# TensorSpeech/TensorFlowASR

Hardware: AMD Instinct MI355X
Metric: audio-hours/sec (train step) Conformer-M RNN-T (higher is better)
Workload: dtype bf16; 1 GPU; Conformer-M transducer full train step (fwd+RNN-T loss+bwd+Adam), LibriSpeech-shaped 16 kHz utterances, 32/GPU, padding=batch, SpecAugment on, dropout 0.1; global_batch=32, parallelism=dp1, params=32461288

## Files before the change

include/tfasr_hip.h:

```cpp
#ifndef TFASR_HIP_H_
#define TFASR_HIP_H_

#include <stddef.h>
#include <stdint.h>

#ifdef __cplusplus
extern "C" {
#endif

#define TFASR_ABI_VERSION 44

typedef enum {
  TFASR_STATUS_SUCCESS = 0,
  TFASR_STATUS_INVALID_VALUE = 1,
  TFASR_STATUS_EXECUTION_FAILED = 2,
  TFASR_STATUS_UNSUPPORTED = 3
} tfasr_status_t;

typedef enum { TFASR_F32 = 0, TFASR_BF16 = 1 } tfasr_dtype_t;

const char* tfasr_status_string(int status);
int tfasr_abi_version(void);
size_t tfasr_launch_count(void);

// ... 37 lines not shown
  void* prez;
  int M, N, K;
  int lda, ldb, ldd;
  int trans_a, trans_b;
  int nb1, nb2;
  long sA1, sA2, sB1, sB2, sD1, sD2;
  float alpha, beta;
  int act;
  int dact;
  int dtype;
  int out_f32;
  int accumulate;
  int split_k;
  float drop_p;
  long drop_seed;
  float* ws;
  long ws_elems;
  float* colsum;
  float* lse_part; int lse_parts; const int32_t* row_label; float* pick;
  const long* seg_a_off; const long* seg_b_off; int seg_k;
  const float* rgrad_coef;
  const void* bns_x; const float* bns_fin; float* bns_out; int bns_copies;
  int bns_c;
} tfasr_gemm_args;

int tfasr_gemm(const tfasr_gemm_args* args, void* stream);
int tfasr_gemm_group(const tfasr_gemm_args* args, int n, void* stream);

int tfasr_layernorm_fwd(const void* x, const float* gamma, const float* beta, void* y, float* mean, float* rstd,
                        long rows, int C, float eps, int dtype, void* stream);
int tfasr_ffn_fused_fwd(const void* x, const float* gamma, const float* beta, const void* W1, const float* b1, const void* W2,
                        const float* b2, void* y, void* ln, float* mean, float* rstd, void* z, void* h, long rows, int d, int F,
                        float ln_eps, float res_factor, float drop_p, long drop_seed1, long drop_seed2, int dtype, void* stream);
int tfasr_ffn_fused_fwd2(const void* x, const float* gamma, const float* beta, const void* W1, const float* b1, const void* W2,
                         const float* b2, void* y, void* ln, float* mean, float* rstd, void* z, int z_factor, void* h, long rows, int d, int F,
                         float ln_eps, float res_factor, float drop_p, long drop_seed1, long drop_seed2, int dtype, void* stream);
int tfasr_ln_dense_fwd(const void* x, const float* gamma, const float* beta, const void* W, const float* b, void* out, void* ln, float* mean,
                       float* rstd, long rows, int d, int N, float ln_eps, int dtype, void* stream);
int tfasr_layernorm_bwd(const void* dy, const void* x, const float* gamma, const float* mean, const float* rstd,
                        const void* add, void* dx, float* dgamma, float* dbeta, long rows, int C, int dtype,
                        void* stream);
int tfasr_layernorm_bwd_drop(const void* dy, const void* x, const float* gamma, const float* mean, const float* rstd,
                             const void* add, void* dx, float* dgamma, float* dbeta, void* dx_dropped, float drop_p,
                             long drop_seed, long rows, int C, int dtype, void* stream);
int tfasr_layernorm_bwd_part_blocks(long rows, int C, int dtype);
int tfasr_layernorm_bwd_part(const void* dy, const void* x, const float* gamma, const float* mean, const float* rstd, const void* add,
// ... 175 lines not shown
int tfasr_conv1_bwd_weight(const void* x, const void* dy, float* dw, float* db, int B, int T0, int F0, int C,
                           int dtype, void* stream);
int tfasr_conv1_fwd_s2d(const void* x, const float* w, const float* bias, void* y, int B, int T0, int F0, int C, int dtype,
                        void* stream);
int tfasr_conv1_bwd_weight_s2d(const void* x, const void* dy, float* dw, float* db, int B, int T0, int F0, int C, int dtype,
                               void* stream);
int tfasr_conv1_stats(const void* x, const float* w, const float* bias, float* stats, int B, int T0, int F0, int C, int dtype,
                      void* stream);
int tfasr_conv1_bn_apply_s2d(const void* x, const float* w, const float* bias, const float* fin, void* y, int B, int T0, int F0, int C,
                             int dtype, void* stream);
int tfasr_conv1_bn_bwd_stats_s2d(const void* x, const float* w, const float* bias, const float* fin, const void* dy, float* bstats, int B,
                                 int T0, int F0, int C, int dtype, void* stream);
int tfasr_conv1_bn_bwd_apply_s2d(const void* x, const float* w, const float* bias, const float* fin, const float* bstats, float count,
                                 const void* dy, float* dw, float* db, int B, int T0, int F0, int C, int dtype, void* stream);
#define TFASR_CONV1_GRAM_DOUBLES 768
int tfasr_conv1_gram(const void* x, double* gram, int B, int T0, int F0, int dtype, void* stream);
int tfasr_conv1_stats_from_gram(const double* gram, const float* w, const float* bias, float* stats, int C, void* stream);
int tfasr_conv1_bn_bwd_onepass_s2d(const void* x, const float* w, const float* bias, const float* fin, const void* dy, float* bstats,
                                   float* pbuf, int B, int T0, int F0, int C, int dtype, void* stream);
int tfasr_conv1_bn_bwd_finalize(const double* gram, const float* w, const float* bias, const float* fin, const float* bstats, float count,
                                const float* pbuf, float* dw, float* db, int C, void* stream);
int tfasr_halo_zero(void* x, int B, int T2, int F2, int W, int dtype, void* stream);
int tfasr_s2d_edge_zero(void* x, int B, int T1, int F1, int C, int dtype, void* stream);
int tfasr_im2col_3x3s2(const void* x, void* col, int B, int T1, int F1, int C, int dtype, void* stream);
int tfasr_col2im_3x3s2(const void* dcol, void* dx, int B, int T1, int F1, int C, int dtype, void* stream);

int tfasr_logmel(const float* signal, int B, int N, float preemph, const float* window, int frame_len, int frame_step,
                 int nfft, const float* melw, const int32_t* band, int F, float eps, void* out, int T0, int dtype,
                 void* stream);

int tfasr_rows_subsample_fwd(const void* x, void* y, int B, int T, int C, int stride, int dtype, void* stream);
int tfasr_rows_subsample_bwd(const void* dy, void* dx, int B, int T, int C, int stride, int dtype, void* stream);
int tfasr_se_pool(const void* x, const int32_t* lengths, float* pool, int B, int T, int C, int dtype, void* stream);
int tfasr_se_scale_fwd(const void* x, const float* scale, void* y, int B, int T, int C, int dtype, void* stream);
int tfasr_se_scale_bwd_reduce(const void* x, const void* dy, float* dscale, int B, int T, int C, int dtype, void* stream);
int tfasr_se_bwd_apply(const void* dy, const float* scale, const float* dpool, const int32_t* lengths, void* dx, int B, int T,
                       int C, int dtype, void* stream);
int tfasr_add_act_fwd(const void* a, const void* b, void* y, long n, int act, int dtype, void* stream);
int tfasr_add_act_bwd(const void* a, const void* b, const void* dy, void* d, long n, int act, int dtype, void* stream);

int tfasr_ctc_beam_search_host(const float* logits, const int32_t* logit_len, int B, int T, int V, int beam_width,
                               int blank_index, int32_t* tokens, int32_t* tokens_len, float* log_prob);

int tfasr_ctc_beam_search_workspace_size(int B, int T, int V, int beam_width, size_t* bytes);
int tfasr_ctc_beam_search(const void* logits, const int32_t* logit_len, int B, int T, int V, int beam_width, int top_paths,
                          int blank_index, int dtype, int32_t* tokens, int32_t* tokens_len, float* log_prob, void* workspace,
// ... 216 lines not shown
```

tensorflowasr_amd/_lib.py:

```python
import ctypes
import os
from ctypes import POINTER, Structure, c_char_p, c_float, c_int, c_int32, c_long, c_size_t, c_void_p

HERE = os.path.dirname(os.path.abspath(__file__))
LIB_PATH = os.environ.get("TFASR_LIB") or os.path.join(HERE, "lib", "libtfasr_hip.so")

TFASR_F32, TFASR_BF16 = 0, 1
ACT_NONE, ACT_SWISH, ACT_TANH, ACT_SIGMOID, ACT_TANH_OUT, ACT_FACTOR = 0, 1, 2, 3, 4, 5


class TfasrError(RuntimeError):
    pass


class GemmArgs(Structure):
    _fields_ = [
        ("A", c_void_p), ("B", c_void_p), ("D", c_void_p),
        ("bias", c_void_p), ("res", c_void_p), ("dact_z", c_void_p), ("prez", c_void_p),
        ("M", c_int), ("N", c_int), ("K", c_int),
        ("lda", c_int), ("ldb", c_int), ("ldd", c_int),
        ("trans_a", c_int), ("trans_b", c_int),
        ("nb1", c_int), ("nb2", c_int),
        ("sA1", c_long), ("sA2", c_long), ("sB1", c_long), ("sB2", c_long), ("sD1", c_long), ("sD2", c_long),
        ("alpha", c_float), ("beta", c_float),
        ("act", c_int), ("dact", c_int), ("dtype", c_int), ("out_f32", c_int), ("accumulate", c_int), ("split_k", c_int),
        ("drop_p", c_float), ("drop_seed", c_long),
        ("ws", c_void_p), ("ws_elems", c_long), ("colsum", c_void_p),
        ("lse_part", c_void_p), ("lse_parts", c_int), ("row_label", c_void_p), ("pick", c_void_p),
        ("seg_a_off", c_void_p), ("seg_b_off", c_void_p), ("seg_k", c_int),
        ("rgrad_coef", c_void_p),
        ("bns_x", c_void_p), ("bns_fin", c_void_p), ("bns_out", c_void_p), ("bns_copies", c_int), ("bns_c", c_int),
    ]


BLOCK_PARAM_NAMES = [
    "ff1/ln/g", "ff1/ln/b", "ff1/d1/w", "ff1/d1/b", "ff1/d2/w", "ff1/d2/b",
    "ff2/ln/g", "ff2/ln/b", "ff2/d1/w", "ff2/d1/b", "ff2/d2/w", "ff2/d2/b",
    "mhsa/ln/g", "mhsa/ln/b", "mhsa/qkv/w", "mhsa/qkv/b", "mhsa/pos/w", "mhsa/pos/b", "mhsa/o/w", "mhsa/o/b", "/enc/u", "/enc/v",
    "conv/ln/g", "conv/ln/b", "conv/pw1/w", "conv/pw1/b", "conv/dw/w", "conv/dw/b", "conv/bn/g", "conv/bn/b", "conv/pw2/w", "conv/pw2/b",
    "ln/g", "ln/b",
]
PHASE_A, PHASE_B = 1, 2


class BlockCfg(Structure):
    _fields_ = [
        ("B", c_int), ("T", c_int), ("d", c_int), ("H", c_int), ("dh", c_int), ("dff", c_int), ("ksize", c_int),
        ("dtype", c_int), ("training", c_int), ("save", c_int), ("use_mask", c_int), ("force_unfused", c_int), ("world", c_int),
        ("site0", c_int), ("drop_epoch", c_long),
        ("drop_p", c_float), ("ffm_res", c_float), ("mhsa_res", c_float), ("conv_res", c_float), ("ln_eps", c_float), ("bn_eps", c_float),
        ("bn_momentum", c_float),
        ("chunk_size", c_int), ("history_size", c_int), ("dw_norm_layer", c_int), ("dh_logical", c_int),
    ]

# ... 105 lines not shown
```

tensorflowasr_amd/conformer.py:

```python
import math
import os

import numpy as np
import torch

from . import kernels as K
from .base_model import BaseModel
from .kernels import ACT_NONE, ACT_SWISH, ACT_TANH_OUT
from .params import ParamStore
from .schemas import AlignOutput, PredictInput, PredictOutput, RecognizeOutput, TrainData, TrainInput, TrainOutput


class SingleProcess:

    world = 1
    rank = 0

    def allreduce_stats_(self, t):
        return t

    def set_reduce(self, on):
        pass

    def grads_ready(self, lo, hi):
# ... 11 lines not shown
    return (v + 4) // 8 * 8 if v >= 12 else v


class ConformerTransducer(BaseModel):
    def __init__(self, cfg, device=None, dtype=torch.bfloat16, seed=0, dp=None):
        if not torch.cuda.is_available():
            raise K._lib.TfasrError("ConformerTransducer needs an MI355X (HIP) device; there is no CPU fallback")
        self.cfg = cfg
        self.device = torch.device("cuda", torch.cuda.current_device()) if device is None else torch.device(device)
        self.dtype = dtype
        pad = (dtype == torch.bfloat16 and cfg.head_size < 64 and getattr(cfg, "encoder", "conformer") == "conformer"
               and os.environ.get("TFASR_HEAD_PAD", "1") != "0")
        cpad = (dtype == torch.bfloat16 and cfg.filters % 64 != 0 and getattr(cfg, "encoder", "conformer") == "conformer"
                and getattr(cfg, "sub_norm", "batch") == "batch" and os.environ.get("TFASR_FILTER_PAD", "1") != "0")
        self.ps = ParamStore(cfg, self.device, dtype, seed, head_phys=64 if pad else None, filt_phys=-(-cfg.filters // 64) * 64 if cpad else None)
        self.dp = dp or SingleProcess()
        self.blank = cfg.blank
        self.time_reduction_factor = cfg.time_reduction_factor
        self.step = 0
        self._consts = {}
        self._bn1_sums_in_gemm = True
        self._bn_stats_copies = 8
        self._conv1_gram = True
        self._rng = np.random.default_rng([seed + 1000, int(self.dp.rank)])
        prio = -1
        self.pred_stream = torch.cuda.Stream(device=self.device, priority=prio)
        self.use_pred_stream = os.environ.get("TFASR_NO_PRED_STREAM", "0") != "1"
        self._dp_force_split = os.environ.get("TFASR_DP_FORCE_SPLIT", "0") == "1" and not isinstance(self.dp, SingleProcess)
        self._lstm_persist_auto = os.environ.get("TFASR_LSTM_PERSIST") is None
        self.optimizer = dict(beta1=0.9, beta2=0.98, eps=1e-9, weight_decay=1e-6, schedule=dict(
            dmodel=cfg.dmodel, warmup_steps=10000, scale=2.0, max_lr=0.05 / math.sqrt(cfg.dmodel)))
        self.ga_steps = 1
        self.prefetched_inputs = False
        self._ga_count = 0
        self._drop_epoch = 0
        self.native_blocks = os.environ.get("TFASR_NATIVE_BLOCK", "1") != "0"
        self.wgrad_stream = {"0": False, "1": True}.get(os.environ.get("TFASR_WGRAD_STREAM"), None)
        self._wgrad_keep = []
        self._blk_params, self._blk_sizes = {}, {}
        self._zero_pool = {}
        self.block_hoist = {"0": False, "1": True}.get(os.environ.get("TFASR_BLOCK_HOIST"), None)
        self.dpext_aux = True
        self.joint_wgrad_aux = False
        self._aux_pending = False
        if self.device.type != "cuda":
            self.aux_stream = None
# ... 60 lines not shown
            return None
        return K.matmul(dy, W, trans_b=True, alpha=alpha, dact_z=dact_z, dact=dact, drop_p=drop[0], drop_seed=drop[1])

    def _h2d(self, x, dtype=torch.int32):
        t = x if isinstance(x, torch.Tensor) else torch.as_tensor(np.asarray(x))
        t = t.to(dtype)
        if t.device.type == "cpu":
            if self.device.type == "cuda":
                t = t.pin_memory()
            t = t.to(self.device, non_blocking=True)
        return t

    def frontend(self, signals, signals_length, training=False, masks=None):
        c = self.cfg
        window, melw, band = self._frontend_consts()
        feats = K.logmel(signals, window, melw, band, c.frame_step, c.nfft, c.preemphasis, c.epsilon, self.dtype)
        flen = [-(-int(n) // c.frame_step) for n in signals_length]
        if training:
            if masks is None:
                masks = self.draw_specaugment(flen)
            fm, tm = masks
            if fm is not None or tm is not None:
                K.specaugment(feats, None if fm is None else self._h2d(fm), None if tm is None else self._h2d(tm), 0.0)
        return feats, flen

    def draw_specaugment(self, flen):
        c = self.cfg
        fcfg, tcfg = c.freq_masking, c.time_masking
        B = len(flen)
        rng = self._rng
        nf = fcfg.get("num_masks", 0) if fcfg else 0
        nt = tcfg.get("num_masks", 0) if tcfg else 0
        fm = np.zeros((B, nf, 2), np.int32) if nf > 0 else None
        tm = np.zeros((B, nt, 2), np.int32) if nt > 0 else None
        nb = c.num_feature_bins
        rnd, rint = rng.random, rng.integers
        fprob = fcfg.get("prob", 1.0) if fcfg else 1.0
        fmax = max(1, int(fcfg["mask_factor"])) if nf > 0 else 1
        tprob = tcfg.get("prob", 1.0) if tcfg else 1.0
        tup = np.float32(tcfg.get("p_upperbound", 1.0)) if tcfg else np.float32(1.0)
        for b in range(B):
            ln = int(flen[b])
            for k in range(nf):
                do = 1 if rnd() <= fprob else 0
                f = do * min(int(rint(0, fmax)), nb)
                fm[b, k] = (do * int(rint(0, max(1, nb - f))), f)
            if nt > 0:
# ... 105 lines not shown
                gram = K.conv1_gram(feats, torch.empty(K.CONV1_GRAM_DOUBLES, dtype=torch.float64, device=self.device))
                K.conv1_stats_from_gram(gram, w0, b0, stats)
            else:
                K.conv1_stats(feats, w0, b0, stats)
            count0 = B * T1 * F1 * self.dp.world
            self.dp.allreduce_stats_(stats[:2 * C])
            K.bn_finalize(stats, count0, ps.p(nm + "/g"), ps.p(nm + "/b"), fin0, ps.state[nm + "/mm"], ps.state[nm + "/mv"], 0.99, 1e-3, True)
        else:
            count0 = B * T1 * F1
            K.bn_finalize(None, 1, ps.p(nm + "/g"), ps.p(nm + "/b"), fin0, ps.state[nm + "/mm"], ps.state[nm + "/mv"], 0.99, 1e-3, False)
        a1_full, a1 = self._salloc(rows, 4 * C, slack, tag="a1")
        K.conv1_bn_apply_s2d(feats, w0, b0, fin0, a1)
        K.halo_zero(a1, B, T2, F2, 4 * C)
        K.s2d_edge_zero(a1, B, T1, F1, C)
        bn0 = (fin0, count0, gram)
        W = ps.w2d("enc/sub/conv1/w")
        _, o = self._salloc(rows, C, slack, tag="o")
        if self.dtype == torch.float32:
            flat, base = a1_full, slack * 4 * C
            for i in range(9):
                K.gemm(flat[base + shift[i] * 4 * C + blk[i] * C:], W[i * C:(i + 1) * C], o, rows, C, C, 4 * C, C, C,
                       bias=ps.p("enc/sub/conv1/b") if i == 0 else None, accumulate=i > 0)
        else:
            K.gemm(a1, W, o, rows, C, 9 * C, 4 * C, C, C, bias=ps.p("enc/sub/conv1/b"), seg=fwd_a)
        K.halo_zero(o, B, T2, F2, C)
        _, a2 = self._salloc(rows, C, 0)
        _, bn1 = self._bn_fwd(o, "enc/sub/bn1", training, ACT_SWISH, rows=B * T2 * F2, y=a2)
        K.halo_zero(a2, B, T2, F2, C)
        drop = self._drop(0, training)
        d = c.dmodel
        x0 = torch.empty(B * T2, d, dtype=self.dtype, device=self.device)
        a2flat = a2.view(-1)
        K.gemm(a2flat[((F2 + 1) + 1) * C:], ps.w2d("enc/linear/w"), x0, T2, d, F2 * C, (F2 + 1) * C, d, d, bias=ps.p("enc/linear/b"),
               nb1=B, sA=((T2 + 1) * (F2 + 1) * C, 0), sD=(T2 * d, 0), drop_p=drop[0], drop_seed=drop[1])
        elen = [-(-(-(-n // 2)) // 2) for n in flen]
        if ctx is not None:
            ctx["sub"] = dict(s2d=True, feats=feats, bn0=bn0, a1=a1, a1_full=a1_full, o=o, bn1=bn1, a2=a2,
                              dims=(B, T0, F0, T1, F1, T2, F2), drop=drop)
        return x0, T2, elen

    def _subsampling_bwd_s2d(self, dx0, ctx):
        ps, c = self.ps, self.cfg
        s = ctx["sub"]
        B, T0, F0, T1, F1, T2, F2 = s["dims"]
        C, d = ps.filt_phys, c.dmodel
        rows, slack = B * (T2 + 1) * (F2 + 1), F2 + 2
        shift, blk, _, dgrad = self._seg_tables(F2, C)
# ... 1277 lines not shown
```

tensorflowasr_amd/csrc/conv2d.hip:

```cpp
#include "common.h"
#include <type_traits>
#include <algorithm>

namespace {

inline int flat_grid(long n) { return (int)std::max<long>(1, std::min<long>((n + 255) / 256, 256L * 32)); }

__device__ __forceinline__ long s2d_off(int b, int t, int f, int T2, int F2, int C) {
  return ((((long)b * (T2 + 1) + (t >> 1) + 1) * (F2 + 1) + (f >> 1) + 1) * 4 + ((t & 1) * 2 + (f & 1))) * C;
}

template <typename T>
__global__ __launch_bounds__(256) void conv1_fwd_kernel(const T* __restrict__ x, const float* __restrict__ w,
                                                        const float* __restrict__ bias, T* __restrict__ y, int B, int T0,
                                                        int F0, int T1, int F1, int C, int s2d) {
  const int c8n = C / 8;
  const long n8 = (long)B * T1 * F1 * c8n;
  const long i0 = (long)blockIdx.x * blockDim.x + threadIdx.x;
  const long stride = (long)gridDim.x * blockDim.x;
  const int c = (int)(i0 % c8n) * 8;
  float wr[9][8], br[8];
#pragma unroll
  for (int k = 0; k < 8; ++k) br[k] = bias ? bias[c + k] : 0.f;
#pragma unroll
// ... 516 lines not shown
  for (long i = (long)blockIdx.x * blockDim.x + threadIdx.x; i < n; i += (long)gridDim.x * blockDim.x) {
    const int c8 = (int)(i % w8);
    long r = i / w8;
    const int k = (int)(r % per_b), b = (int)(r / per_b);
    const int tt = k <= F2 ? 0 : k - F2, ff = k <= F2 ? k : 0;
    st8(x + (((long)b * (T2 + 1) + tt) * (F2 + 1) + ff) * W + (long)c8 * 8, z);
  }
}
template <typename T>
__global__ __launch_bounds__(256) void s2d_edge_zero_kernel(T* __restrict__ x, int B, int T1, int F1, int T2, int F2, int C) {
  const int c8n = C / 8;
  const int nt = (T1 & 1) ? F2 * 2 : 0;
  const int nf = (F1 & 1) ? T2 * 2 : 0;
  const long n = (long)B * (nt + nf) * c8n;
  const float z[8] = {0, 0, 0, 0, 0, 0, 0, 0};
  for (long i = (long)blockIdx.x * blockDim.x + threadIdx.x; i < n; i += (long)gridDim.x * blockDim.x) {
    const int c8 = (int)(i % c8n);
    long r = i / c8n;
    const int k = (int)(r % (nt + nf)), b = (int)(r / (nt + nf));
    int tt, ff, blk;
    if (k < nt) { tt = T2; ff = 1 + (k >> 1); blk = 2 + (k & 1); }
    else { const int q = k - nt; tt = 1 + (q >> 1); ff = F2; blk = (q & 1) * 2 + 1; }
    st8(x + ((((long)b * (T2 + 1) + tt) * (F2 + 1) + ff) * 4 + blk) * C + (long)c8 * 8, z);
  }
}

}

#define DISPATCH_T(dtype, CALL_F32, CALL_BF16) \
  do { if ((dtype) == TFASR_F32) { CALL_F32; } else if ((dtype) == TFASR_BF16) { CALL_BF16; } else return TFASR_STATUS_INVALID_VALUE; } while (0)

static int conv1_fwd_impl(const void* x, const float* w, const float* bias, void* y, int B, int T0, int F0, int C,
                          int dtype, void* stream_, int s2d) {
  if (!x || !w || !y || B <= 0 || T0 <= 0 || F0 <= 0 || C <= 0 || C % 8) return TFASR_STATUS_INVALID_VALUE;
  const int T1 = (T0 + 1) / 2, F1 = (F0 + 1) / 2;
  hipStream_t s = (hipStream_t)stream_;
  if (C == 256 && F0 + 2 <= 260) {
    const int g2 = std::min(B * T1, 8192);
    DISPATCH_T(dtype,
               TFASR_KLAUNCH(conv1_fwd_rows_kernel<float>, dim3(g2), dim3(256), 0, s, (const float*)x, w, bias, (float*)y, B, T0, F0, T1, F1, s2d),
               TFASR_KLAUNCH(conv1_fwd_rows_kernel<bf16_t>, dim3(g2), dim3(256), 0, s, (const bf16_t*)x, w, bias, (bf16_t*)y, B, T0, F0, T1, F1, s2d));
    TFASR_CHECK_LAUNCH();
    return TFASR_STATUS_SUCCESS;
  }
  int grid = flat_grid((long)B * T1 * F1 * C / 8);
  if ((256 % (C / 8)) != 0) {
// ... 138 lines not shown

extern "C" int tfasr_halo_zero(void* x, int B, int T2, int F2, int W, int dtype, void* stream_) {
  if (!x || B <= 0 || T2 <= 0 || F2 <= 0 || W <= 0 || W % 8) return TFASR_STATUS_INVALID_VALUE;
  hipStream_t s = (hipStream_t)stream_;
  const int grid = flat_grid((long)B * ((F2 + 1) + T2) * (W / 8));
  DISPATCH_T(dtype, TFASR_KLAUNCH(halo_zero_kernel<float>, dim3(grid), dim3(256), 0, s, (float*)x, B, T2, F2, W),
             TFASR_KLAUNCH(halo_zero_kernel<bf16_t>, dim3(grid), dim3(256), 0, s, (bf16_t*)x, B, T2, F2, W));
  TFASR_CHECK_LAUNCH();
  return TFASR_STATUS_SUCCESS;
}

extern "C" int tfasr_s2d_edge_zero(void* x, int B, int T1, int F1, int C, int dtype, void* stream_) {
  if (!x || B <= 0 || T1 <= 0 || F1 <= 0 || C <= 0 || C % 8) return TFASR_STATUS_INVALID_VALUE;
  if (!(T1 & 1) && !(F1 & 1)) return TFASR_STATUS_SUCCESS;
  const int T2 = (T1 + 1) / 2, F2 = (F1 + 1) / 2;
  hipStream_t s = (hipStream_t)stream_;
  const int grid = flat_grid((long)B * (((T1 & 1) ? F2 * 2 : 0) + ((F1 & 1) ? T2 * 2 : 0)) * (C / 8));
  DISPATCH_T(dtype, TFASR_KLAUNCH(s2d_edge_zero_kernel<float>, dim3(grid), dim3(256), 0, s, (float*)x, B, T1, F1, T2, F2, C),
             TFASR_KLAUNCH(s2d_edge_zero_kernel<bf16_t>, dim3(grid), dim3(256), 0, s, (bf16_t*)x, B, T1, F1, T2, F2, C));
  TFASR_CHECK_LAUNCH();
  return TFASR_STATUS_SUCCESS;
}

extern "C" int tfasr_im2col_3x3s2(const void* x, void* col, int B, int T1, int F1, int C, int dtype, void* stream_) {
  if (!x || !col || B <= 0 || T1 <= 0 || F1 <= 0 || C <= 0 || C % 8) return TFASR_STATUS_INVALID_VALUE;
  const int T2 = (T1 + 1) / 2, F2 = (F1 + 1) / 2;
  hipStream_t s = (hipStream_t)stream_;
  const int grid = flat_grid((long)B * T2 * F2 * 9 * C / 8);
  DISPATCH_T(dtype,
             TFASR_KLAUNCH(im2col_kernel<float>, dim3(grid), dim3(256), 0, s, (const float*)x, (float*)col, B, T1, F1, T2, F2, C),
             TFASR_KLAUNCH(im2col_kernel<bf16_t>, dim3(grid), dim3(256), 0, s, (const bf16_t*)x, (bf16_t*)col, B, T1, F1, T2, F2, C));
  TFASR_CHECK_LAUNCH();
  return TFASR_STATUS_SUCCESS;
}

extern "C" int tfasr_col2im_3x3s2(const void* dcol, void* dx, int B, int T1, int F1, int C, int dtype, void* stream_) {
  if (!dcol || !dx || B <= 0 || T1 <= 0 || F1 <= 0 || C <= 0 || C % 8) return TFASR_STATUS_INVALID_VALUE;
  const int T2 = (T1 + 1) / 2, F2 = (F1 + 1) / 2;
  hipStream_t s = (hipStream_t)stream_;
  const int grid = flat_grid((long)B * T1 * F1 * C / 8);
  DISPATCH_T(dtype,
             TFASR_KLAUNCH(col2im_kernel<float>, dim3(grid), dim3(256), 0, s, (const float*)dcol, (float*)dx, B, T1, F1, T2, F2, C),
             TFASR_KLAUNCH(col2im_kernel<bf16_t>, dim3(grid), dim3(256), 0, s, (const bf16_t*)dcol, (bf16_t*)dx, B, T1, F1, T2, F2, C));
  TFASR_CHECK_LAUNCH();
  return TFASR_STATUS_SUCCESS;
}
// ... 1 lines not shown
```

tensorflowasr_amd/csrc/gemm.hip:

```cpp
#include "common.h"
#include <stdlib.h>

namespace {

constexpr int BM = 128, BN = 128;

template <typename T> struct Cfg;
template <> struct Cfg<bf16_t> { static constexpr int BK = 64, LD = 72; };
template <> struct Cfg<float>  { static constexpr int BK = 16, LD = 17; };

__device__ __forceinline__ bool aligned16(const void* p) { return (((uintptr_t)p) & 15) == 0; }

__device__ __forceinline__ void load_direct(bf16_t* s, const bf16_t* g, long ld, int rows0, int nrows_total,
                                            int kt, int k_end) {
  constexpr int BK = Cfg<bf16_t>::BK, LD = Cfg<bf16_t>::LD;
  for (int c = threadIdx.x; c < BM * BK / 8; c += 256) {
    const int row = c / (BK / 8), kc = (c % (BK / 8)) * 8;
    const int gr = rows0 + row, gk = kt + kc;
    uint4 v = make_uint4(0, 0, 0, 0);
    if (gr < nrows_total) {
      const bf16_t* p = g + (long)gr * ld + gk;
      if (gk + 8 <= k_end && aligned16(p)) v = *reinterpret_cast<const uint4*>(p);
      else {
        uint32_t w[4] = {0, 0, 0, 0};
// ... 366 lines not shown
        if (st != TFASR_STATUS_SUCCESS) return st;
      }
    } else if (st != TFASR_STATUS_SUCCESS) {
      return st;
    }
    i += m;
  }
  return TFASR_STATUS_SUCCESS;
}

extern "C" int tfasr_gemm(const tfasr_gemm_args* args, void* stream_) {
  if (!args || !args->A || !args->B || (!args->D && !args->lse_part)) return TFASR_STATUS_INVALID_VALUE;
  tfasr_gemm_args a = *args;
  if (a.rgrad_coef && (!a.row_label || !a.D || a.lse_part)) return TFASR_STATUS_INVALID_VALUE;
  if (a.M <= 0 || a.N <= 0 || a.K <= 0) return TFASR_STATUS_INVALID_VALUE;
  if (a.nb1 < 1) a.nb1 = 1;
  if (a.nb2 < 1) a.nb2 = 1;
  if (a.split_k < 1) a.split_k = 1;
  if (a.accumulate && !a.out_f32) return TFASR_STATUS_INVALID_VALUE;
  if (a.split_k > 1 && !a.accumulate) return TFASR_STATUS_INVALID_VALUE;
  if (a.split_k > 1 && (a.res || a.dact_z || a.prez || a.act != TFASR_ACT_NONE || a.drop_p > 0.f)) return TFASR_STATUS_INVALID_VALUE;
  if (a.drop_p < 0.f || a.drop_p >= 1.f) return TFASR_STATUS_INVALID_VALUE;
  if (a.colsum && !(a.accumulate && a.trans_a && !a.trans_b && a.nb1 * a.nb2 == 1)) return TFASR_STATUS_INVALID_VALUE;
  hipStream_t stream = (hipStream_t)stream_;
  if (a.dtype == TFASR_BF16 && use_fast_path()) {
    const int st = tfasr_gemm_fast_try(a, stream);
    if (st != TFASR_STATUS_UNSUPPORTED) return st;
  }
  if (a.lse_part || a.rgrad_coef || a.bns_out) return TFASR_STATUS_UNSUPPORTED;
  if (a.seg_a_off) return TFASR_STATUS_UNSUPPORTED;
  if (a.colsum) {
    const int st = tfasr_colsum(a.B, a.ldb, a.colsum, a.K, a.N, a.alpha, a.dtype, stream_);
    if (st != TFASR_STATUS_SUCCESS) return st;
    a.colsum = nullptr;
  }
  if (a.dtype == TFASR_BF16) return launch<bf16_t>(a, stream);
  if (a.dtype == TFASR_F32) return launch<float>(a, stream);
  return TFASR_STATUS_INVALID_VALUE;
}
```

tensorflowasr_amd/csrc/gemm_big.h:

```cpp

template <bool ACC>
__device__ __forceinline__ void mfma_acc(float4_t& c, const short8_t& a, const short8_t& b) {
  if constexpr (ACC) asm volatile("v_mfma_f32_16x16x32_bf16 %0, %1, %2, %0" : "+a"(c) : "v"(a), "v"(b));
  else asm volatile("v_mfma_f32_16x16x32_bf16 %0, %1, %2, %0" : "+v"(c) : "v"(a), "v"(b));
}

__device__ __forceinline__ short8_t frag_trans_big(const char* sB, uint32_t tb, int j, int kk) {
  const char* q = sB + ((tb ^ (uint32_t)(j << 5)) + (uint32_t)(kk * 32 * 512));
  const short4_t lo = __builtin_amdgcn_ds_read_tr16_b64_v4i16((__attribute__((address_space(3))) short4_t*)(q));
  const short4_t hi = __builtin_amdgcn_ds_read_tr16_b64_v4i16((__attribute__((address_space(3))) short4_t*)(q + 4 * 512));
  short8_t v;
  v[0] = lo[0]; v[1] = lo[1]; v[2] = lo[2]; v[3] = lo[3];
  v[4] = hi[0]; v[5] = hi[1]; v[6] = hi[2]; v[7] = hi[3];
  return v;
}

template <bool TB, int BN_, int EPI, bool SEG, bool TR = false>
__global__ __launch_bounds__(512) __attribute__((amdgpu_waves_per_eu(2, 2)))
void gemm_big_kernel(const tfasr_gemm_args p, const int gx, const int gy, const int ntiles) {
  constexpr bool C_LSE = (EPI & E_LSE) != 0;
  static_assert(!TR || (BN_ == 256 && (EPI & ~(E_LSE | E_DACT)) == 0), "transposed accumulators: 256 columns; plain / log-softmax / tanh-out epilogues");
  static_assert(!TR || !((EPI & E_LSE) && (EPI & E_DACT)), "statistics and tanh-out never meet");
#ifdef TFASR_BIG_ASM_DMA
  constexpr bool ASM_DMA = TFASR_BIG_ASM_DMA != 0;
// ... 31 lines not shown
    __syncthreads();
  }
  struct Tile { int m0, m0s, n0, n0s, ok; uint32_t offA[2]; uint32_t offB[2]; };
  auto tile_of = [&](int it) {
    Tile T;
    T.ok = 0;
    int t;
    if ((G & 7) == 0) {
      const int x = bid & 7, slot = bid >> 3, round0 = it * G, R = ntiles - round0;
      if (R <= 0) return T;
      if (R >= G) t = round0 + x * (G >> 3) + slot;
      else {
        const int q = R >> 3, rem = R & 7;
        if (slot >= q + (x < rem ? 1 : 0)) return T;
        t = round0 + (x < rem ? x * (q + 1) : rem * (q + 1) + (x - rem) * q) + slot;
      }
    } else {
      if (it > 0) return T;
      t = bid;
    }
    const int tx = t % gx, ty = t / gx;
    T.ok = 1;
    T.m0 = ty * BMB;
    T.m0s = min(T.m0, p.M - BMB);
    T.n0 = tx * BN_;
    T.n0s = TB ? min(T.n0, p.N - BN_) : T.n0;
    int lt = lane;
    asm volatile("" : "+v"(lt));
#pragma unroll
    for (int par = 0; par < 2; ++par) {
      const int row = (w * NA + par) * 8 + (lt >> 3), pc = lt & 7;
      T.offA[par] = (uint32_t)(((long)row * p.lda + ((pc ^ key_d(row)) << 3)) * 2);
      if constexpr (TB) {
        const int rowb = (w * NB + par) * 8 + (lt >> 3);
        T.offB[par] = (uint32_t)(((long)rowb * p.ldb + ((pc ^ key_d(rowb)) << 3)) * 2);
      } else {
        constexpr int CPR = BN_ / 8, KPI = 64 / CPR;
        const int maxchunk = ((p.N + 7) >> 3) - 1;
        const int k = (w * NB + par) * KPI + lt / CPR, pcb = lt % CPR;
        const int c = min((T.n0 >> 3) + (pcb ^ key_t(k)), maxchunk);
        T.offB[par] = (uint32_t)(((long)k * p.ldb + ((long)c << 3)) * 2);
      }
    }
    return T;
  };
  const int nfull = p.K / BK;
// ... 522 lines not shown
    if (!nxt.ok) break;
    if constexpr (ALIAS) {
      __syncthreads();
      if (nsl > 1 && grpB) { issue_half(nxt, 1, 1, 0); if (SCHED == 1) issue_half(nxt, 1, 1, 1); }
    }
    __builtin_amdgcn_s_waitcnt(0x0F70);
    cur = nxt;
  }
}

int g_gemm_big_mode = -1;

template <bool TB>
int launch_big(const tfasr_gemm_args& a, bool generic, int need, bool tanh_out, hipStream_t stream) {
  static const bool env_off = false;
  const bool off = g_gemm_big_mode < 0 ? env_off : g_gemm_big_mode == 0;
  if (off || generic || need != 0 || a.accumulate || a.split_k > 1 || a.nb1 * a.nb2 != 1 || a.colsum || a.out_f32 || a.K < 2 * BK || (a.K & 7) || a.M < 256 || (TB && (a.N & 7))) return TFASR_STATUS_UNSUPPORTED;
  const bool seg = a.seg_a_off != nullptr;
  if (seg && !(a.seg_k > 0 && (a.seg_k % BK) == 0 && (a.K % a.seg_k) == 0 && a.K / BK <= 64)) return TFASR_STATUS_UNSUPPORTED;
  int bn = 0;
  if (TB && !seg && !a.lse_part && (a.N % 320) == 0) bn = 320;
  else if (a.N >= (TB ? 256 : 192) && ((a.N % 256) == 0 || (a.N % 256) >= 192)) bn = 256;
  if (!bn) return TFASR_STATUS_UNSUPPORTED;
  const int gx = (a.N + bn - 1) / bn, gy = (a.M + 255) / 256;
  const long ntiles = (long)gx * gy;
  static const long min_tiles = 2L * num_cus();
  if (ntiles < min_tiles || ntiles > 0x7fffffffL) return TFASR_STATUS_UNSUPPORTED;
  if (tanh_out && (!TB || seg || a.lse_part)) return TFASR_STATUS_UNSUPPORTED;
  if (a.lse_part && !(a.row_label && a.pick && bn == 256 && a.lse_parts == ((a.N + 127) / 128) * 2)) return TFASR_STATUS_UNSUPPORTED;
  if (a.rgrad_coef && (TB || seg || tanh_out || bn != 256 || !a.row_label)) return TFASR_STATUS_UNSUPPORTED;
  if (!a.D && !a.lse_part) return TFASR_STATUS_UNSUPPORTED;
  const int ncu = num_cus();
  const int G = ntiles >= ncu ? (ncu & ~7) : (int)ntiles;
  auto go = [&](auto kern, int smem) {
    static bool attr_done = false;
    if (!attr_done) { hipFuncSetAttribute((const void*)kern, hipFuncAttributeMaxDynamicSharedMemorySize, smem); attr_done = true; }
    TFASR_KLAUNCH(kern, dim3(G), dim3(512), smem, stream, a, gx, gy, (int)ntiles);
  };
  constexpr int S256 = 2 * (256 * BK * 2 + 256 * BK * 2) + 8 * 8 * 68 * 4;
  constexpr int S320 = 2 * (256 * BK * 2 + 320 * BK * 2);
  static const bool tr_on = !(false);
  const bool tr = tr_on && (a.ldd & 7) == 0 && (a.N & 7) == 0 && (((uintptr_t)a.D) & 15) == 0;
  if (tanh_out) {
    if constexpr (TB) {
      if (bn == 320) go(gemm_big_kernel<true, 320, E_DACT, false>, S320);
      else { if (tr) go(gemm_big_kernel<true, 256, E_DACT, false, true>, S256); else go(gemm_big_kernel<true, 256, E_DACT, false>, S256); }
    } else return TFASR_STATUS_UNSUPPORTED;
  } else if (bn == 320) {
    if constexpr (TB) go(gemm_big_kernel<true, 320, 0, false>, S320);
    else return TFASR_STATUS_UNSUPPORTED;
// ... 15 lines not shown
```

tensorflowasr_amd/csrc/gemm_fast.hip:

```cpp
#include "common.h"
#include <type_traits>
#include <string.h>
#include <stdlib.h>

typedef __attribute__((ext_vector_type(4))) short short4_t;

#ifdef TFASR_GEMM_TIMING
__device__ long long g_gemm_timing[16 * 32768];
#endif

namespace {

constexpr int BM = 128, BK = 64;
constexpr int A_BYTES = BM * BK * 2;

#define LDS_PTR(p) ((__attribute__((address_space(3))) void*)(p))
#define GLB_PTR(p) ((const __attribute__((address_space(1))) void*)(p))

__device__ __forceinline__ uint32_t lds_u32(const char* s) {
  return (uint32_t)__builtin_amdgcn_readfirstlane((int)(uint32_t)(uintptr_t)s);
}
__device__ __forceinline__ void glds16(const void* g, const char* lds_uniform) {
#ifdef TFASR_GLDS_BUILTIN
  __builtin_amdgcn_global_load_lds(GLB_PTR(g), LDS_PTR(lds_uniform), 16, 0, 0);
// ... 243 lines not shown
        const int round0 = it * G, R = ntiles - round0, slot = bid >> 3;
        if (R <= 0) return T;
        int t;
        if (R >= G) t = round0 + x * (G >> 3) + slot;
        else {
          const int q = R >> 3, rem = R & 7;
          if (slot >= q + (x < rem ? 1 : 0)) return T;
          t = round0 + (x < rem ? x * (q + 1) : rem * (q + 1) + (x - rem) * q) + slot;
        }
        tx = t % gx; const int rest = t / gx; ty = rest % gy; tz = rest / gy;
      }
    } else {
      if (it > 0) return T;
      const int q = G >> 3, rem = G & 7, xcd = bid & 7, slot = bid >> 3;
      const int t = G >= 16 ? (xcd < rem ? xcd * (q + 1) : rem * (q + 1) + (xcd - rem) * q) + slot : (int)bid;
      tx = t % gx; const int rest = t / gx; ty = rest % gy; tz = rest / gy;
    }
    const int ks = tz % split, bidx = tz / split;
    const int b1 = bidx / p.nb2, b2 = bidx % p.nb2;
    T.A = (const bf16_t*)p.A + b1 * p.sA1 + b2 * p.sA2;
    T.B = (const bf16_t*)p.B + b1 * p.sB1 + b2 * p.sB2;
    T.doff = b1 * p.sD1 + b2 * p.sD2;
    T.m0 = ty * BM;
    T.n0 = tx * BN;
    T.ks = ks;
    T.k_begin = ks * kchunk;
    T.k_end = min(p.K, T.k_begin + kchunk);
    const int len = max(T.k_end - T.k_begin, 0);
    T.nfull = len / BK;
    T.tail = (len % BK) != 0;
    if (TA) prep_trans<128>(T.sa, T.A, p.lda, T.m0, p.M, T.k_begin, w, lane); else prep_direct<128>(T.sa, T.A, p.lda, T.m0, p.M, T.k_begin, w, lane);
    if (TB) prep_direct<BN_>(T.sb, T.B, p.ldb, T.n0, p.N, T.k_begin, w, lane); else prep_trans<BN_>(T.sb, T.B, p.ldb, T.n0, p.N, T.k_begin, w, lane);
    return T;
  };
  const long stepA = TA ? (long)BK * p.lda : (long)BK, stepB = TB ? (long)BK : (long)BK * p.ldb;
  auto issue = [&](const Tile& T, int slab, int stage) {
    char* sA = smem + stage * STAGE_BYTES;
    char* sB = sA + A_BYTES;
    if constexpr (SEG) {
      issue_from<128>(sA, T.sa, seg_tab[0][slab], w);
      issue_from<BN_>(sB, T.sb, seg_tab[1][slab], w);
    } else {
      issue_from<128>(sA, T.sa, slab * stepA, w);
      issue_from<BN_>(sB, T.sb, slab * stepB, w);
    }
  };
// ... 569 lines not shown
  if (narrow) {
    if (!generic && need == 0) return launch_epi<TA, TB, 64, 0>(a, grid, stream);
    if constexpr (!TA && !TB) {
      if (!generic && need == E_RES) return launch_epi<TA, TB, 64, E_RES>(a, grid, stream);
      if (!generic && need == (E_RES | E_DROP)) return launch_epi<TA, TB, 64, E_RES | E_DROP>(a, grid, stream);
    }
    if (t128 > num_cus() && a.N > 64 && !generic) {
      if constexpr (!TA && !TB) {
        if (need == E_ACT) return launch_epi<TA, TB, 64, E_ACT>(a, grid, stream);
        if (need == (E_ACT | E_DROP)) return launch_epi<TA, TB, 64, E_ACT | E_DROP>(a, grid, stream);
      }
      if constexpr (!TA && TB) {
        if (need == E_DACT) return launch_epi<TA, TB, 64, E_DACT>(a, grid, stream);
        if (need == (E_DACT | E_DROP)) return launch_epi<TA, TB, 64, E_DACT | E_DROP>(a, grid, stream);
        if (need == E_MUL) return launch_epi<TA, TB, 64, E_MUL>(a, grid, stream);
      }
    }
    return launch_epi<TA, TB, 64, E_GEN>(a, grid, stream);
  }
  if (a.seg_a_off) {
    if constexpr (!TA) {
      if (!generic && need == 0 && !a.accumulate && split == 1 && a.nb1 * a.nb2 == 1 && a.seg_k > 0 && (a.seg_k % BK) == 0 && (a.K % a.seg_k) == 0 &&
          a.K / BK <= 64 && !a.lse_part) {
        dim3 g128((a.N + 127) / 128, (a.M + BM - 1) / BM, 1);
        const long ntiles = (long)g128.x * g128.y;
        const int slots = 2 * num_cus();
        int G = (int)(ntiles < slots ? ntiles : slots);
        if (ntiles >= slots) G &= ~7;
        constexpr int SMEM = 2 * (A_BYTES + 128 * BK * 2) + 4 * (64 / (128 / 16)) * (128 / 2 + 4) * 4;
        TFASR_KLAUNCH((gemm_seg_kernel<TA, TB>), dim3(G), dim3(256), SMEM, stream, a, (int)g128.x, (int)g128.y, 1, (int)ntiles);
        TFASR_CHECK_LAUNCH();
        return TFASR_STATUS_SUCCESS;
      }
    }
    return TFASR_STATUS_UNSUPPORTED;
  }
  if (a.lse_part) {
    if constexpr (!TA && !TB) {
      if (!generic && need == 0 && !a.accumulate && a.nb1 * a.nb2 == 1 && a.row_label && a.pick && a.lse_parts == ((a.N + 127) / 128) * 2)
        return launch_epi<TA, TB, 128, E_LSE>(a, grid, stream);
    }
    return TFASR_STATUS_UNSUPPORTED;
  }
  if (!generic) {
    if (need == 0) return launch_epi<TA, TB, 128, 0>(a, grid, stream);
    if constexpr (!TA && !TB) {
      if (need == E_RES) return launch_epi<TA, TB, 128, E_RES>(a, grid, stream);
// ... 184 lines not shown
```

tensorflowasr_amd/kernels.py:

```python
import ctypes
import os

import torch

from . import _lib
from ._lib import ACT_FACTOR, ACT_NONE, ACT_SIGMOID, ACT_SWISH, ACT_TANH, ACT_TANH_OUT, TFASR_BF16, TFASR_F32, GemmArgs, check

_WS_CACHE = {}
_SPLITK_WS = False


def _dt(t):
    if t.dtype == torch.float32:
        return TFASR_F32
    if t.dtype == torch.bfloat16:
        return TFASR_BF16
    raise TypeError(f"unsupported activation dtype {t.dtype}")


def _p(t):
    if t is None:
        return None
    if not t.is_cuda:
        raise _lib.TfasrError("tensorflowasr_amd ops need HIP device tensors (no CPU fallback on the product path)")
# ... 198 lines not shown
    _edit_check(_lib.load().tfasr_edit_distance_workspace_size(P, N, M, ctypes.byref(n)), "edit_distance_workspace_size")
    return n.value


def edit_distance(hyp, ref, hyp_len=None, ref_len=None, skip_id=-1):
    for t in (hyp, ref, hyp_len, ref_len):
        if t is not None and not t.is_cuda:
            raise _lib.TfasrError("tensorflowasr_amd ops need HIP device tensors (no CPU fallback on the product path)")
    assert hyp.dim() == 2 and ref.dim() == 2 and hyp.shape[0] == ref.shape[0] and hyp.dtype == torch.int32 and ref.dtype == torch.int32
    P, N, M = hyp.shape[0], hyp.shape[1], ref.shape[1]
    for ln in (hyp_len, ref_len):
        assert ln is None or (ln.dtype == torch.int32 and ln.shape == (P,))
    counts = torch.empty(P, 5, dtype=torch.int32, device=hyp.device)
    if P == 0:
        return counts
    ws = workspace(edit_distance_workspace_size(P, N, M), hyp.device, "edit")
    _edit_check(_lib.load().tfasr_edit_distance(_p(hyp) if N else _p(counts), _p(hyp_len), _p(ref) if M else _p(counts), _p(ref_len), P, N, M,
                                                 int(skip_id), _p(counts), _p(ws), ws.numel(), _stream()), "edit_distance")
    return counts


def gemm(A, B, out, M, N, K, lda, ldb, ldd, trans_a=False, trans_b=False, bias=None, res=None, dact_z=None,
         prez=None, alpha=1.0, beta=1.0, act=ACT_NONE, dact=ACT_NONE, nb1=1, nb2=1, sA=(0, 0), sB=(0, 0), sD=(0, 0),
         accumulate=False, split_k=1, drop_p=0.0, drop_seed=0, colsum=None, lse=None, seg=None, rgrad=None, bns=None):
    a = _gemm_args(A, B, out, M, N, K, lda, ldb, ldd, trans_a, trans_b, bias, res, dact_z, prez, alpha, beta, act, dact, nb1, nb2, sA, sB, sD,
                   accumulate, split_k, drop_p, drop_seed, colsum)
    if rgrad is not None:
        coef, row_label = rgrad
        assert coef.dtype == torch.float32 and coef.is_contiguous() and row_label.dtype == torch.int32
        a.rgrad_coef, a.row_label = coef.data_ptr(), row_label.data_ptr()
    if seg is not None:
        a.seg_a_off, a.seg_b_off, a.seg_k = seg[0].data_ptr(), (seg[1].data_ptr() if seg[1] is not None else None), int(seg[2])
        assert seg[0].dtype == torch.int64 and seg[0].is_cuda
    if bns is not None:
        bx, bfin, bout = bns[:3]
        bc = int(bns[3]) if len(bns) > 3 else N
        assert bfin.dtype == torch.float32 and bout.dtype == torch.float32 and bout.is_contiguous()
        a.bns_x, a.bns_fin, a.bns_out, a.bns_copies = bx.data_ptr(), bfin.data_ptr(), bout.data_ptr(), bout.numel() // (2 * bc)
        a.bns_c = 0 if bc == N else bc
    if lse is not None:
        part, row_label, pick = lse
        assert part.dtype == torch.float32 and pick.dtype == torch.float32 and row_label.dtype == torch.int32
        a.lse_part, a.lse_parts, a.row_label, a.pick = part.data_ptr(), part.shape[1], row_label.data_ptr(), pick.data_ptr()
    st = _lib.load().tfasr_gemm(ctypes.byref(a), _stream())
    if (lse is not None or seg is not None or rgrad is not None or bns is not None) and st == _lib.STATUS_UNSUPPORTED:
        raise _lib.TfasrUnsupported("gemm: fused row statistics / K-segments / gradient epilogue are not available for this product")
    check(st, "gemm")
    return out


def gemm_group(calls):
    arr = (GemmArgs * len(calls))()
    for i, kw in enumerate(calls):
        arr[i] = _gemm_args(**kw)
    check(_lib.load().tfasr_gemm_group(arr, len(calls), _stream()), "gemm_group")

# ... 625 lines not shown

def conv1_stats_from_gram(gram, w, bias, stats):
    check(_L().tfasr_conv1_stats_from_gram(_p(gram), _p(w), _p(bias), _p(stats), w.shape[-1], _stream()), "conv1_stats_from_gram")


def conv1_bn_bwd_onepass_s2d(x, w, bias, fin, dy, bstats, pbuf):
    B, T0, F0 = x.shape[:3]
    check(_L().tfasr_conv1_bn_bwd_onepass_s2d(_p(x), _p(w), _p(bias), _p(fin), _p(dy), _p(bstats), _p(pbuf), B, T0, F0, w.shape[-1], _dt(x),
                                              _stream()), "conv1_bn_bwd_onepass")


def conv1_bn_bwd_finalize(gram, w, bias, fin, bstats, count, pbuf, dw, db):
    check(_L().tfasr_conv1_bn_bwd_finalize(_p(gram), _p(w), _p(bias), _p(fin), _p(bstats), float(count), _p(pbuf), _p(dw), _p(db), w.shape[-1],
                                           _stream()), "conv1_bn_bwd_finalize")


def halo_zero(x, B, T2, F2, W):
    check(_L().tfasr_halo_zero(_p(x), B, T2, F2, W, _dt(x), _stream()), "halo_zero")
    return x


def s2d_edge_zero(x, B, T1, F1, C):
    check(_L().tfasr_s2d_edge_zero(_p(x), B, T1, F1, C, _dt(x), _stream()), "s2d_edge_zero")
    return x


def im2col_3x3s2(x, col=None):
    B, T1, F1, C = x.shape
    T2, F2 = (T1 + 1) // 2, (F1 + 1) // 2
    if col is None:
        col = torch.empty(B * T2 * F2, 9 * C, dtype=x.dtype, device=x.device)
    check(_L().tfasr_im2col_3x3s2(_p(x), _p(col), B, T1, F1, C, _dt(x), _stream()), "im2col")
    return col


def col2im_3x3s2(dcol, B, T1, F1, C):
    dx = torch.empty(B, T1, F1, C, dtype=dcol.dtype, device=dcol.device)
    check(_L().tfasr_col2im_3x3s2(_p(dcol), _p(dx), B, T1, F1, C, _dt(dcol), _stream()), "col2im")
    return dx


def logmel(signal, window, melw, band, frame_step, nfft, preemph, eps, out_dtype):
    B, N = signal.shape
    T0 = -(-N // frame_step)
    F = melw.shape[1]
    out = torch.empty(B, T0, F, dtype=out_dtype, device=signal.device)
# ... 970 lines not shown
```

Before: 4.820 audio-hours/sec.

## Skip padded-tail row tiles in subsampling conv1 GEMM and replicate tail rows

On the host, each utterance's padded tail in the subsampled grid is computed from its signal length and SpecAugment time masks. The first subsampling conv GEMM is then launched only over row tiles that touch real frames. A new kernel fills the skipped tail tiles by copying a representative padded row per utterance, since padded input gives identical outputs. This saves MMA work on padding, but adds host-side table building and a per-step host-to-device upload, and it only kicks in when enough tiles can be skipped.

```diff
diff --git a/include/tfasr_hip.h b/include/tfasr_hip.h
--- a/include/tfasr_hip.h
+++ b/include/tfasr_hip.h
@@ -83,6 +83,7 @@
   const float* rgrad_coef;
   const void* bns_x; const float* bns_fin; float* bns_out; int bns_copies;
   int bns_c;
+  const int32_t* row_tiles; int n_row_tiles;
 } tfasr_gemm_args;
 
 int tfasr_gemm(const tfasr_gemm_args* args, void* stream);
@@ -304,6 +305,8 @@
                                 const float* pbuf, float* dw, float* db, int C, void* stream);
 int tfasr_halo_zero(void* x, int B, int T2, int F2, int W, int dtype, void* stream);
 int tfasr_s2d_edge_zero(void* x, int B, int T1, int F1, int C, int dtype, void* stream);
+int tfasr_s2d_tail_fill(void* x, const int32_t* tiles, int n_tiles, const int32_t* rep_tt, int B, int T2, int F2, int C, int dtype,
+                        void* stream);
 int tfasr_im2col_3x3s2(const void* x, void* col, int B, int T1, int F1, int C, int dtype, void* stream);
 int tfasr_col2im_3x3s2(const void* dcol, void* dx, int B, int T1, int F1, int C, int dtype, void* stream);
 
diff --git a/tensorflowasr_amd/_lib.py b/tensorflowasr_amd/_lib.py
--- a/tensorflowasr_amd/_lib.py
+++ b/tensorflowasr_amd/_lib.py
@@ -30,6 +30,7 @@
         ("seg_a_off", c_void_p), ("seg_b_off", c_void_p), ("seg_k", c_int),
         ("rgrad_coef", c_void_p),
         ("bns_x", c_void_p), ("bns_fin", c_void_p), ("bns_out", c_void_p), ("bns_copies", c_int), ("bns_c", c_int),
+        ("row_tiles", c_void_p), ("n_row_tiles", c_int),
     ]
 
 
diff --git a/tensorflowasr_amd/conformer.py b/tensorflowasr_amd/conformer.py
--- a/tensorflowasr_amd/conformer.py
+++ b/tensorflowasr_amd/conformer.py
@@ -57,6 +57,8 @@
         self._bn1_sums_in_gemm = True
         self._bn_stats_copies = 8
         self._conv1_gram = True
+        self._sub_tail_once = os.environ.get("TFASR_SUB_TAIL", "1") != "0"
+        self._front_tail = None
         self._rng = np.random.default_rng([seed + 1000, int(self.dp.rank)])
         prio = -1
         self.pred_stream = torch.cuda.Stream(device=self.device, priority=prio)
@@ -163,7 +165,58 @@
             fm, tm = masks
             if fm is not None or tm is not None:
                 K.specaugment(feats, None if fm is None else self._h2d(fm), None if tm is None else self._h2d(tm), 0.0)
+        self._front_tail = (feats, self._feature_tail(signals_length, masks[1] if training else None))
         return feats, flen
+
+    def _feature_tail(self, signals_length, tm):
+        step = self.cfg.frame_step
+        tf = -(-(np.asarray([int(n) for n in signals_length], dtype=np.int64) + 1) // step)
+        if tm is not None:
+            if not isinstance(tm, torch.Tensor) or tm.device.type != "cpu":
+                return None
+            m = tm.numpy().astype(np.int64)
+            if m.shape[1] > 0:
+                tf = np.maximum(tf, (m[:, :, 0] + m[:, :, 1]).max(axis=1))
+        return tuple(int(v) for v in tf)
+
+    @staticmethod
+    def _tail_rows(tf, T0):
+        tf = np.asarray(tf, dtype=np.int64)
+        t1c = (tf + 1) // 2 + 1
+        a1 = (t1c + 1) // 2 + 1
+        return dict(feats=tf, a1=a1, o=a1 + 1, a2=a1 + 1)
+
+    @classmethod
+    def _tail_blocks(cls, tf, B, T0, T2, F2):
+        rep = cls._tail_rows(tf, T0)["o"]
+        has = rep + 1 <= T2
+        rep = np.where(has, rep, 1)
+        end = np.where(has, rep + 1, T2 + 1)
+        nblk = -(-(B * (T2 + 1) * (F2 + 1)) // 256)
+        base = np.arange(B, dtype=np.int64) * (T2 + 1)
+        lo = (base + 1) * (F2 + 1) // 256
+        hi = ((base + end) * (F2 + 1) - 1) // 256
+        mark = np.zeros(nblk + 1, np.int64)
+        np.add.at(mark, lo, 1)
+        np.add.at(mark, hi + 1, -1)
+        real = np.cumsum(mark[:nblk]) > 0
+        return np.flatnonzero(real), np.flatnonzero(~real), rep
+
+    def _tail_tables(self, tf, B, T0, T2, F2):
+        key = ("tail", tf, T0, F2)
+        hit = self._consts.get(key, 0)
+        if hit != 0:
+            return hit
+        comp, skip, rep = self._tail_blocks(tf, B, T0, T2, F2)
+        out = None
+        if skip.size * 16 >= comp.size + skip.size:
+            dev = self._h2d(np.concatenate([comp, skip, rep]).astype(np.int32))
+            out = (dev[:comp.size], dev[comp.size:comp.size + skip.size], dev[comp.size + skip.size:])
+        old = [k for k in self._consts if isinstance(k, tuple) and k[:1] == ("tail",)]
+        for k in old[:max(0, len(old) - 7)]:
+            del self._consts[k]
+        self._consts[key] = out
+        return out
 
     def draw_specaugment(self, flen):
         c = self.cfg
@@ -315,7 +368,17 @@
                 K.gemm(flat[base + shift[i] * 4 * C + blk[i] * C:], W[i * C:(i + 1) * C], o, rows, C, C, 4 * C, C, C,
                        bias=ps.p("enc/sub/conv1/b") if i == 0 else None, accumulate=i > 0)
         else:
-            K.gemm(a1, W, o, rows, C, 9 * C, 4 * C, C, C, bias=ps.p("enc/sub/conv1/b"), seg=fwd_a)
+            tail, ft, self._front_tail = None, self._front_tail, None
+            if self._sub_tail_once and ft is not None and ft[0] is feats and ft[1] is not None and len(ft[1]) == B:
+                tail = self._tail_tables(ft[1], B, T0, T2, F2)
+            if tail is not None:
+                try:
+                    K.gemm(a1, W, o, rows, C, 9 * C, 4 * C, C, C, bias=ps.p("enc/sub/conv1/b"), seg=fwd_a, row_tiles=tail[0])
+                    K.s2d_tail_fill(o, tail[1], tail[2], B, T2, F2, C)
+                except K._lib.TfasrUnsupported:
+                    tail = None
+            if tail is None:
+                K.gemm(a1, W, o, rows, C, 9 * C, 4 * C, C, C, bias=ps.p("enc/sub/conv1/b"), seg=fwd_a)
         K.halo_zero(o, B, T2, F2, C)
         _, a2 = self._salloc(rows, C, 0)
         _, bn1 = self._bn_fwd(o, "enc/sub/bn1", training, ACT_SWISH, rows=B * T2 * F2, y=a2)
diff --git a/tensorflowasr_amd/csrc/conv2d.hip b/tensorflowasr_amd/csrc/conv2d.hip
--- a/tensorflowasr_amd/csrc/conv2d.hip
+++ b/tensorflowasr_amd/csrc/conv2d.hip
@@ -562,6 +562,23 @@
     if (k < nt) { tt = T2; ff = 1 + (k >> 1); blk = 2 + (k & 1); }
     else { const int q = k - nt; tt = 1 + (q >> 1); ff = F2; blk = (q & 1) * 2 + 1; }
     st8(x + ((((long)b * (T2 + 1) + tt) * (F2 + 1) + ff) * 4 + blk) * C + (long)c8 * 8, z);
+  }
+}
+
+__global__ __launch_bounds__(256) void s2d_tail_fill_kernel(uint4* __restrict__ x, const int32_t* __restrict__ tiles, const int32_t* __restrict__ rep_tt,
+                                                            int T2, int F2, int c8n, long rows) {
+  const long nblk = (rows + 255) / 256;
+  const long tile = min(max((long)tiles[blockIdx.x >> 2], 0L), nblk - 1);
+  const long r0 = tile * 256 + (blockIdx.x & 3) * 64;
+  const int per_b = (T2 + 1) * (F2 + 1);
+  for (int i = threadIdx.x; i < 64 * c8n; i += 256) {
+    const long row = r0 + i / c8n;
+    if (row >= rows) break;
+    const int c8 = i % c8n;
+    const int b = (int)(row / per_b), ff = (int)(row % (F2 + 1));
+    const int rt = min(max(rep_tt[b], 1), T2);
+    const long src = ((long)b * (T2 + 1) + rt) * (F2 + 1) + ff;
+    if (src != row) x[row * c8n + c8] = x[src * c8n + c8];
   }
 }
 
@@ -746,6 +763,18 @@
   return TFASR_STATUS_SUCCESS;
 }
 
+extern "C" int tfasr_s2d_tail_fill(void* x, const int32_t* tiles, int n_tiles, const int32_t* rep_tt, int B, int T2, int F2, int C, int dtype,
+                                   void* stream_) {
+  if (!x || !tiles || !rep_tt || B <= 0 || T2 <= 0 || F2 <= 0 || C <= 0 || n_tiles < 0) return TFASR_STATUS_INVALID_VALUE;
+  const long rows = (long)B * (T2 + 1) * (F2 + 1);
+  if (n_tiles > (rows + 255) / 256) return TFASR_STATUS_INVALID_VALUE;
+  if (dtype != TFASR_BF16 || C % 8 || (((uintptr_t)x) & 15)) return TFASR_STATUS_UNSUPPORTED;
+  if (n_tiles == 0) return TFASR_STATUS_SUCCESS;
+  TFASR_KLAUNCH(s2d_tail_fill_kernel, dim3(4 * n_tiles), dim3(256), 0, (hipStream_t)stream_, (uint4*)x, tiles, rep_tt, T2, F2, C / 8, rows);
+  TFASR_CHECK_LAUNCH();
+  return TFASR_STATUS_SUCCESS;
+}
+
 extern "C" int tfasr_im2col_3x3s2(const void* x, void* col, int B, int T1, int F1, int C, int dtype, void* stream_) {
   if (!x || !col || B <= 0 || T1 <= 0 || F1 <= 0 || C <= 0 || C % 8) return TFASR_STATUS_INVALID_VALUE;
   const int T2 = (T1 + 1) / 2, F2 = (F1 + 1) / 2;
diff --git a/tensorflowasr_amd/csrc/gemm.hip b/tensorflowasr_amd/csrc/gemm.hip
--- a/tensorflowasr_amd/csrc/gemm.hip
+++ b/tensorflowasr_amd/csrc/gemm.hip
@@ -412,6 +412,10 @@
   if (a.split_k > 1 && (a.res || a.dact_z || a.prez || a.act != TFASR_ACT_NONE || a.drop_p > 0.f)) return TFASR_STATUS_INVALID_VALUE;
   if (a.drop_p < 0.f || a.drop_p >= 1.f) return TFASR_STATUS_INVALID_VALUE;
   if (a.colsum && !(a.accumulate && a.trans_a && !a.trans_b && a.nb1 * a.nb2 == 1)) return TFASR_STATUS_INVALID_VALUE;
+  if (a.row_tiles) {
+    if (a.n_row_tiles <= 0 || a.n_row_tiles > (a.M + 255) / 256) return TFASR_STATUS_INVALID_VALUE;
+    if (!a.seg_a_off || a.trans_a || a.accumulate || a.split_k > 1 || a.nb1 * a.nb2 != 1 || a.dtype != TFASR_BF16) return TFASR_STATUS_UNSUPPORTED;
+  }
   hipStream_t stream = (hipStream_t)stream_;
   if (a.dtype == TFASR_BF16 && use_fast_path()) {
     const int st = tfasr_gemm_fast_try(a, stream);
diff --git a/tensorflowasr_amd/csrc/gemm_big.h b/tensorflowasr_amd/csrc/gemm_big.h
--- a/tensorflowasr_amd/csrc/gemm_big.h
+++ b/tensorflowasr_amd/csrc/gemm_big.h
@@ -77,6 +77,7 @@
     const int tx = t % gx, ty = t / gx;
     T.ok = 1;
     T.m0 = ty * BMB;
+    if constexpr (SEG) { if (p.row_tiles) T.m0 = min(max(p.row_tiles[ty], 0), (p.M + BMB - 1) / BMB - 1) * BMB; }
     T.m0s = min(T.m0, p.M - BMB);
     T.n0 = tx * BN_;
     T.n0s = TB ? min(T.n0, p.N - BN_) : T.n0;
@@ -645,10 +646,11 @@
   if (TB && !seg && !a.lse_part && (a.N % 320) == 0) bn = 320;
   else if (a.N >= (TB ? 256 : 192) && ((a.N % 256) == 0 || (a.N % 256) >= 192)) bn = 256;
   if (!bn) return TFASR_STATUS_UNSUPPORTED;
-  const int gx = (a.N + bn - 1) / bn, gy = (a.M + 255) / 256;
-  const long ntiles = (long)gx * gy;
+  int gx = (a.N + bn - 1) / bn, gy = (a.M + 255) / 256;
+  long ntiles = (long)gx * gy;
   static const long min_tiles = 2L * num_cus();
   if (ntiles < min_tiles || ntiles > 0x7fffffffL) return TFASR_STATUS_UNSUPPORTED;
+  if (a.row_tiles) { gy = a.n_row_tiles; ntiles = (long)gx * gy; }
   if (tanh_out && (!TB || seg || a.lse_part)) return TFASR_STATUS_UNSUPPORTED;
   if (a.lse_part && !(a.row_label && a.pick && bn == 256 && a.lse_parts == ((a.N + 127) / 128) * 2)) return TFASR_STATUS_UNSUPPORTED;
   if (a.rgrad_coef && (TB || seg || tanh_out || bn != 256 || !a.row_label)) return TFASR_STATUS_UNSUPPORTED;
diff --git a/tensorflowasr_amd/csrc/gemm_fast.hip b/tensorflowasr_amd/csrc/gemm_fast.hip
--- a/tensorflowasr_amd/csrc/gemm_fast.hip
+++ b/tensorflowasr_amd/csrc/gemm_fast.hip
@@ -289,6 +289,7 @@
     T.B = (const bf16_t*)p.B + b1 * p.sB1 + b2 * p.sB2;
     T.doff = b1 * p.sD1 + b2 * p.sD2;
     T.m0 = ty * BM;
+    if constexpr (SEG) { if (p.row_tiles) T.m0 = min(max(p.row_tiles[ty >> 1], 0) * 256 + (ty & 1) * BM, ((p.M + BM - 1) / BM - 1) * BM); }
     T.n0 = tx * BN;
     T.ks = ks;
     T.k_begin = ks * kchunk;
@@ -904,7 +905,7 @@
     if constexpr (!TA) {
       if (!generic && need == 0 && !a.accumulate && split == 1 && a.nb1 * a.nb2 == 1 && a.seg_k > 0 && (a.seg_k % BK) == 0 && (a.K % a.seg_k) == 0 &&
           a.K / BK <= 64 && !a.lse_part) {
-        dim3 g128((a.N + 127) / 128, (a.M + BM - 1) / BM, 1);
+        dim3 g128((a.N + 127) / 128, a.row_tiles ? 2 * a.n_row_tiles : (a.M + BM - 1) / BM, 1);
         const long ntiles = (long)g128.x * g128.y;
         const int slots = 2 * num_cus();
         int G = (int)(ntiles < slots ? ntiles : slots);
diff --git a/tensorflowasr_amd/kernels.py b/tensorflowasr_amd/kernels.py
--- a/tensorflowasr_amd/kernels.py
+++ b/tensorflowasr_amd/kernels.py
@@ -244,7 +244,7 @@
 
 def gemm(A, B, out, M, N, K, lda, ldb, ldd, trans_a=False, trans_b=False, bias=None, res=None, dact_z=None,
          prez=None, alpha=1.0, beta=1.0, act=ACT_NONE, dact=ACT_NONE, nb1=1, nb2=1, sA=(0, 0), sB=(0, 0), sD=(0, 0),
-         accumulate=False, split_k=1, drop_p=0.0, drop_seed=0, colsum=None, lse=None, seg=None, rgrad=None, bns=None):
+         accumulate=False, split_k=1, drop_p=0.0, drop_seed=0, colsum=None, lse=None, seg=None, rgrad=None, bns=None, row_tiles=None):
     a = _gemm_args(A, B, out, M, N, K, lda, ldb, ldd, trans_a, trans_b, bias, res, dact_z, prez, alpha, beta, act, dact, nb1, nb2, sA, sB, sD,
                    accumulate, split_k, drop_p, drop_seed, colsum)
     if rgrad is not None:
@@ -254,6 +254,9 @@
     if seg is not None:
         a.seg_a_off, a.seg_b_off, a.seg_k = seg[0].data_ptr(), (seg[1].data_ptr() if seg[1] is not None else None), int(seg[2])
         assert seg[0].dtype == torch.int64 and seg[0].is_cuda
+    if row_tiles is not None:
+        assert seg is not None and row_tiles.dtype == torch.int32 and row_tiles.is_cuda and row_tiles.is_contiguous()
+        a.row_tiles, a.n_row_tiles = row_tiles.data_ptr(), row_tiles.numel()
     if bns is not None:
         bx, bfin, bout = bns[:3]
         bc = int(bns[3]) if len(bns) > 3 else N
@@ -925,6 +928,14 @@
 
 def s2d_edge_zero(x, B, T1, F1, C):
     check(_L().tfasr_s2d_edge_zero(_p(x), B, T1, F1, C, _dt(x), _stream()), "s2d_edge_zero")
+
+
+def s2d_tail_fill(x, tiles, rep_tt, B, T2, F2, C):
+    assert tiles.dtype == torch.int32 and rep_tt.dtype == torch.int32 and tiles.is_cuda and rep_tt.is_cuda and rep_tt.numel() == B
+    st = _L().tfasr_s2d_tail_fill(_p(x), _p(tiles), tiles.numel(), _p(rep_tt), B, T2, F2, C, _dt(x), _stream())
+    if st == _lib.STATUS_UNSUPPORTED:
+        raise _lib.TfasrUnsupported("s2d_tail_fill: bf16 tensors with C % 8 == 0 only")
+    check(st, "s2d_tail_fill")
     return x
 
 
```

Measured after the change: 4.869 audio-hours/sec (median of 6 runs). +1.0%, better.
